# NVIDIA/audio-flamingo

Measured on AMD Instinct MI355X. Metric: audio-sec/s + decoder tokens/s, AF3-7B bf16 train, higher is better.
Workload: dtype bf16; 1 GPU; AF3 (AF-Whisper 32L + Qwen2.5-7B 28L, MLP projector) bf16 train step fwd+bwd+AdamW, 30 s clips, S=1024; micro_batch_per_gpu=8, global_batch=8, seq_len=1024, parallelism=dp1, activation_checkpointing=False

## Files before the change

### audio-flamingo_amd/csrc/attention_lds.hip

```cpp
#include "common.h"
#include "../../include/afk.h"

#ifdef AFK_PROBES
#define AFK_DBG(p) ((p).dbg)
#else
#define AFK_DBG(p) 0
#endif

namespace {

struct AttnArgs2 {
    const bf16* Q; int64_t q_bs, q_hs, q_rs;
    const bf16* K; int64_t k_bs, k_hs, k_rs;
    const bf16* V; int64_t v_bs, v_hs, v_rs;
    bf16* O; int64_t o_bs, o_hs, o_rs;
    const bf16* dO; int64_t do_bs, do_hs, do_rs;
    bf16* dQ; int64_t dq_bs, dq_hs, dq_rs;
    bf16* dK; int64_t dk_bs, dk_hs, dk_rs;
    bf16* dV; int64_t dv_bs, dv_hs, dv_rs;
    float* LSE;
    const float* delta;
    const int* kv_len;
    const int* kv_lo;
    int B, Hq, Hkv, S, Spad;
// ... 13 lines not shown
};

typedef __attribute__((address_space(3))) void lds_void;
typedef const __attribute__((address_space(1))) void gbl_void;
typedef __attribute__((address_space(3))) bf16x4 lds_bf16x4;

constexpr float NEG_INF = -INFINITY;
#define MFMA(a, b, c) __builtin_amdgcn_mfma_f32_32x32x16_bf16(a, b, c, 0, 0, 0)
#define ROW_OF(r, hi) (((r) & 3) + 8 * ((r) >> 2) + 4 * (hi))

__device__ __forceinline__ f32x16 zero16() {
    f32x16 z;
#pragma unroll
    for (int i = 0; i < 16; ++i) z[i] = 0.f;
    return z;
}

__device__ __forceinline__ float other_half(float x) {
    const unsigned u = __float_as_uint(x);
    const auto r = __builtin_amdgcn_permlane32_swap(u, u, false, false);
    return (threadIdx.x & 32) ? __uint_as_float(r[0]) : __uint_as_float(r[1]);
}
constexpr float LOG2E = 1.4426950408889634f, LN2 = 0.6931471805599453f;

template <bool WIDE>
__device__ __forceinline__ void store_block32(bf16* rowp, const f32x16& acc, float mul, int hi) {
    if constexpr (WIDE) {
#pragma unroll
        for (int t = 0; t < 2; ++t) {
            bf16x8 o;
#pragma unroll
            for (int e = 0; e < 4; ++e) {
                const auto r = __builtin_amdgcn_permlane32_swap(__float_as_uint(acc[8 * t + e]), __float_as_uint(acc[8 * t + 4 + e]), false, false);
                o[e] = (bf16)(__uint_as_float(r[0]) * mul);
                o[4 + e] = (bf16)(__uint_as_float(r[1]) * mul);
            }
            *(bf16x8*)(rowp + 16 * t + 8 * hi) = o;
        }
    } else {
#pragma unroll
        for (int qd = 0; qd < 4; ++qd) {
            bf16x4 o;
#pragma unroll
            for (int e = 0; e < 4; ++e) o[e] = (bf16)(acc[4 * qd + e] * mul);
            *(bf16x4*)(rowp + 8 * qd + 4 * hi) = o;
        }
// ... 140 lines not shown

#define AFK_ATTN_BARRIER()                                    \
    do {                                                      \
        asm volatile("s_waitcnt vmcnt(0)" ::: "memory");      \
        __builtin_amdgcn_sched_barrier(0);                    \
        __builtin_amdgcn_s_barrier();                         \
        __builtin_amdgcn_sched_barrier(0);                    \
    } while (0)
#define AFK_ATTN_BARRIER_P(p_)                                \
    do {                                                      \
        if (AFK_DBG(p_) & 16) {    \
            asm volatile("s_waitcnt vmcnt(0)" ::: "memory");  \
            __builtin_amdgcn_sched_barrier(0);                \
        } else if (AFK_DBG(p_) & 2) {                         \
            __builtin_amdgcn_sched_barrier(0);                \
            __builtin_amdgcn_s_barrier();                     \
            __builtin_amdgcn_sched_barrier(0);                \
        } else {                                              \
            AFK_ATTN_BARRIER();                               \
        }                                                     \
    } while (0)
constexpr float RESCALE_THR = 8.f;

template <int D, bool LM, int SCH>
__global__ __launch_bounds__(256, 2) void attn_fwd_lds_kernel(AttnArgs2 p) {
    using T = Tile<D>;
    constexpr int KS = T::KS, DT = T::DT;
    extern __shared__ __attribute__((aligned(16))) char smem[];
    const int lane = threadIdx.x & 63;
    const int wave = __builtin_amdgcn_readfirstlane(threadIdx.x >> 6);
    const int l31 = lane & 31, hi = lane >> 5;
    const typename T::Offs offs = T::make_offs(lane);
    const QBlock blk = attn_qblock(p);
    const int b = blk.b, h = blk.h, hk = h / (p.Hq / p.Hkv);
    const int qb0 = blk.z * 128;
    const int q0 = qb0 + wave * 32;
    const int q = q0 + l31;
    const int qc = min(q, p.S - 1);
    const int kv_len = p.kv_len ? min(p.kv_len[b], p.S) : p.S;
    const int kv_lo = p.kv_lo ? min(max(p.kv_lo[b], 0), kv_len) : 0;

    const bf16* Qp = p.Q + b * p.q_bs + h * p.q_hs + (int64_t)qc * p.q_rs + hi * 8;
    bf16x8 qf[KS];
#pragma unroll
    for (int ks = 0; ks < KS; ++ks) qf[ks] = *(const bf16x8*)(Qp + ks * 16);

    const bf16* Kbase = p.K + b * p.k_bs + hk * p.k_hs;
// ... 125 lines not shown
        float mx = fmaxf(st[0][0], st[1][0]);
#pragma unroll
        for (int r = 1; r < 16; ++r) mx = fmaxf(fmaxf(mx, st[0][r]), st[1][r]);
        mx = fmaxf(mx, other_half(mx)) * c2;
        if (__builtin_expect(__builtin_amdgcn_ballot_w64(mx > m + RESCALE_THR) != 0, 0)) {
            asm volatile("" ::);
            const float m_new = fmaxf(m, mx);
            const float alpha = __builtin_amdgcn_exp2f(m - ((m_new == NEG_INF) ? 0.f : m_new));
            if (LM) lacc[0] *= alpha;
            else l *= alpha;
#pragma unroll
            for (int dt = 0; dt < DT; ++dt)
#pragma unroll
                for (int r = 0; r < 16; ++r) oacc[dt][r] *= alpha;
            m = m_new;
        }
        const float nm = (m == NEG_INF) ? 0.f : -m;
        const f32x2 c2v = {c2, c2}, nmv = {nm, nm};
        f32x2 rs2 = {0.f, 0.f};
#pragma unroll
        for (int kt2 = 0; kt2 < 2; ++kt2)
#pragma unroll
            for (int r = 0; r < 16; r += 2) {
                const f32x2 s2 = {st[kt2][r], st[kt2][r + 1]};
                const f32x2 t2 = __builtin_elementwise_fma(s2, c2v, nmv);
                const f32x2 p2 = {__builtin_amdgcn_exp2f(t2[0]), __builtin_amdgcn_exp2f(t2[1])};
                if (!LM) rs2 += p2;
                pb[2 * kt2 + (r >> 3)][r & 7] = (bf16)p2[0];
                pb[2 * kt2 + (r >> 3)][(r & 7) + 1] = (bf16)p2[1];
            }
        if (!LM) l += rs2[0] + rs2[1];
        }
        if (LM) {
#pragma unroll
            for (int s4 = 0; s4 < 4; ++s4) lacc = MFMA(ones, pb[s4], lacc);
        }
        afk_frag_ring<DT>(issue, [&](auto g_, bf16x8(&f)[4]) {
            constexpr int dt = decltype(g_)::value;
#pragma unroll
            for (int s4 = 0; s4 < 4; ++s4) oacc[dt] = MFMA(f[s4], pb[s4], oacc[dt]);
        }, fa, fb);
    };

    const int j0 = kv_lo >> 6, j_int0 = (kv_lo + 63) >> 6;
    if (ntiles > j0) stage(j0);
    AFK_ATTN_BARRIER();
#pragma unroll
    for (int ks = 0; ks < KS; ++ks) asm volatile("" : "+v"(qf[ks]));
    int j = j0;
    constexpr std::false_type NO_DMA{};
// ... 242 lines not shown
            else l += other_half(l);
            const float inv = (l > 0.f) ? 1.f / l : 0.f;
            bf16* Op = p.O + bcur * p.o_bs + hcur * p.o_hs + (int64_t)qcur * p.o_rs;
            if (p.wide) {
#pragma unroll
                for (int dt = 0; dt < DT; ++dt) store_block32<true>(Op + dt * 32, oacc[dt], inv, hi);
            } else {
#pragma unroll
                for (int dt = 0; dt < DT; ++dt) store_block32<false>(Op + dt * 32, oacc[dt], inv, hi);
            }
            if (hi == 0 && p.LSE) p.LSE[((int64_t)bcur * p.Hq + hcur) * p.Spad + qcur] = (l > 0.f) ? -(m + __log2f(l)) / c2 : INFINITY;
        }
        if (!has_next) break;
    }
    if (threadIdx.x == 0 && !p.paired) {
        const int gone = __hip_atomic_fetch_add(queue + 1, 1, __ATOMIC_RELAXED, __HIP_MEMORY_SCOPE_AGENT);
        if (gone == (int)gridDim.x - 1) {
            __hip_atomic_store(queue, 0, __ATOMIC_RELAXED, __HIP_MEMORY_SCOPE_AGENT);
            __hip_atomic_store(queue + 1, 0, __ATOMIC_RELAXED, __HIP_MEMORY_SCOPE_AGENT);
        }
    }
}

template <int D, int SCH>
__global__ __launch_bounds__(256, 2) void attn_bwd_dq_lds_kernel(AttnArgs2 p) {
    using T = Tile<D>;
    constexpr int KS = T::KS, DT = T::DT;
    extern __shared__ __attribute__((aligned(16))) char smem[];
    const int lane = threadIdx.x & 63;
    const int wave = __builtin_amdgcn_readfirstlane(threadIdx.x >> 6);
    const int l31 = lane & 31, hi = lane >> 5;
    const typename T::Offs offs = T::make_offs(lane);
    const QBlock blk = attn_qblock(p);
    const int b = blk.b, h = blk.h, hk = h / (p.Hq / p.Hkv);
    const int qb0 = blk.z * 128;
    const int q0 = qb0 + wave * 32;
    const int q = q0 + l31;
    const int qc = min(q, p.S - 1);
    const int kv_len = p.kv_len ? min(p.kv_len[b], p.S) : p.S;
    const int kv_lo = p.kv_lo ? min(max(p.kv_lo[b], 0), kv_len) : 0;

    const bf16* Qp = p.Q + b * p.q_bs + h * p.q_hs + (int64_t)qc * p.q_rs + hi * 8;
    const bf16* dOp = p.dO + b * p.do_bs + h * p.do_hs + (int64_t)qc * p.do_rs + hi * 8;
    bf16x8 qf[KS], dof[KS];
#pragma unroll
    for (int ks = 0; ks < KS; ++ks) {
        qf[ks] = *(const bf16x8*)(Qp + ks * 16);
// ... 68 lines not shown
        constexpr bool isv = (i & 1) != 0;
        const uint32_t dst = lds0 + (jn & 1) * 2 * T::BYTES + wave * 1024 + (isv ? T::BYTES : 0) + 4 * u0 * 1024;
        if constexpr (isv) afk_dma16_saddr(Vbase + ((int64_t)jn * 64 + u0 * 4 * T::RPU) * p.v_rs, voff[0], dst);
        else afk_dma16_saddr(Kbase + ((int64_t)jn * 64 + u0 * 4 * T::RPU) * p.k_rs, koff[0], dst);
    };
    auto tile = [&](int j, auto masked_, auto par_, auto dma_) {
        constexpr bool MASKED = decltype(masked_)::value;
        constexpr bool DMA = decltype(dma_)::value;
        constexpr int POFF = par_static_off<decltype(par_)>(2 * T::BYTES);
        const uint32_t boff = par_dyn_off(par_, 2 * T::BYTES);
        const char* kimg = smem + POFF + boff;
        const char* vimg = kimg + T::BYTES;
        bf16x8 fa[4], fb[4];
        auto issue = [&](auto g_, bf16x8(&dst)[4]) {
            constexpr int dt = decltype(g_)::value;
            const uint32_t a0 = ktr[dt][0] + boff, a1 = ktr[dt][1] + boff;
            afk_static_for<4>([&](auto s_) { constexpr int s4 = decltype(s_)::value; dst[s4] = afk_lds_tr_frag<POFF + s4 * 16 * T::RS>(a0, a1); });
        };
        const f32x2 c2v = {c2, c2}, nl = {nlse, nlse}, nd = {ndlt, ndlt};
        bf16x8 dsb[4];
        auto ds_half = [&](int kt2, const f32x16& sh, const f32x16& dh) {
#pragma unroll
            for (int r = 0; r < 16; r += 2) {
                const f32x2 s2 = {sh[r], sh[r + 1]};
                const f32x2 t2 = __builtin_elementwise_fma(s2, c2v, nl);
                const f32x2 p2 = {__builtin_amdgcn_exp2f(t2[0]), __builtin_amdgcn_exp2f(t2[1])};
                const f32x2 d2 = {dh[r], dh[r + 1]};
                f32x2 ds2 = p2 * (d2 + nd);
                if (MASKED) {
                    const int key = j * 64 + kt2 * 32 + ROW_OF(r, hi);
                    if ((key >= kv_len) || (key < kv_lo) || (p.causal && key > q)) ds2[0] = 0.f;
                    if ((key + 1 >= kv_len) || (key + 1 < kv_lo) || (p.causal && key + 1 > q)) ds2[1] = 0.f;
                }
                dsb[2 * kt2 + (r >> 3)][r & 7] = (bf16)ds2[0];
                dsb[2 * kt2 + (r >> 3)][(r & 7) + 1] = (bf16)ds2[1];
            }
        };
        if constexpr (SCH == 0) {
            f32x16 st[2] = {zero16(), zero16()}, dp[2] = {zero16(), zero16()};
#pragma unroll
            for (int ks = 0; ks < KS; ++ks) {
                st[0] = MFMA(T::row_frag(kimg, offs, 0, ks), qf[ks], st[0]);
                st[1] = MFMA(T::row_frag(kimg, offs, 1, ks), qf[ks], st[1]);
                dp[0] = MFMA(T::row_frag(vimg, offs, 0, ks), dof[ks], dp[0]);
                dp[1] = MFMA(T::row_frag(vimg, offs, 1, ks), dof[ks], dp[1]);
            }
            issue(std::integral_constant<int, 0>{}, fa);
            ds_half(0, st[0], dp[0]);
            ds_half(1, st[1], dp[1]);
        } else {
            constexpr int NGK = KS / 2, NT = 2 * NGK, PPG = (2 * NP + NT - 1) / NT;
// ... 83 lines not shown
    if (q < p.S) {
        bf16* dQp = p.dQ + b * p.dq_bs + h * p.dq_hs + (int64_t)q * p.dq_rs;
        float mul = p.scale;
        if (p.rope_cos) {
            if (p.rope_cos_lanes && !p.rope_pos) {
                const int64_t rb = (int64_t)(q0 >> 5) * 32 * D;
                rope_bwd_rows<DT, true>(dqacc, mul, p.rope_cos_lanes + rb, p.rope_sin_lanes + rb, hi, l31);
            } else {
                const int64_t pr = p.rope_pos ? p.rope_pos[(int64_t)b * p.S + q] : q;
                rope_bwd_rows<DT>(dqacc, mul, p.rope_cos + pr * D, p.rope_sin + pr * D, hi);
            }
            mul = 1.f;
        }
        if (p.wide) {
#pragma unroll
            for (int dt = 0; dt < DT; ++dt) store_block32<true>(dQp + dt * 32, dqacc[dt], mul, hi);
        } else {
#pragma unroll
            for (int dt = 0; dt < DT; ++dt) store_block32<false>(dQp + dt * 32, dqacc[dt], mul, hi);
        }
    }
}

template <int D>
__global__ __launch_bounds__(256, (D <= 64 ? 2 : 1)) void attn_bwd_dkdv_lds_kernel(AttnArgs2 p) {
    using T = Tile<D>;
    constexpr int KS = T::KS, DT = T::DT;
    extern __shared__ __attribute__((aligned(16))) char smem[];
    uint64_t rt_entry = 0, rt1 = 0;
    if (AFK_DBG(p) & 4) asm volatile("s_memrealtime %0\n s_waitcnt lgkmcnt(0)" : "=s"(rt_entry)::"memory");
    const int lane = threadIdx.x & 63;
    const int wave = __builtin_amdgcn_readfirstlane(threadIdx.x >> 6);
    const int l31 = lane & 31, hi = lane >> 5;
    const typename T::Offs offs = T::make_offs(lane);
    const int b = blockIdx.y, group = p.Hq / p.Hkv;
    const int hy = blockIdx.x;
    const int P = p.split_heads;
    const int hk = P ? hy / P : hy;
    const int g_begin = P ? ((hy % P) * group) / P : 0;
    const int g_count = P ? (((hy % P) + 1) * group) / P - g_begin : group;
    const int kb0 = blockIdx.z * 128;
    const int key0 = kb0 + wave * 32;
    const int key = key0 + l31;
    const int keyc = min(key, p.S - 1);
    const int kv_len = p.kv_len ? min(p.kv_len[b], p.S) : p.S;
    const int kv_lo = p.kv_lo ? min(max(p.kv_lo[b], 0), kv_len) : 0;
    const bool wave_live = key0 < p.S;
// ... 50 lines not shown
            const uint32_t dst = lds0 + slot * BUF + wave * 1024;
#pragma unroll
            for (int u0 = 0; u0 < NP; ++u0) {
                afk_dma16_saddr(q0, qoff[u0], dst + 4 * u0 * 1024);
                afk_dma16_saddr(d0, dooff[u0], dst + T::BYTES + 4 * u0 * 1024);
            }
        } else {
            T::stage(buf, qb, p.q_rs, qt * 64, p.S - 1, wave, lane);
            T::stage(buf + T::BYTES, dob, p.do_rs, qt * 64, p.S - 1, wave, lane);
        }
        if (wave == 0)
            __builtin_amdgcn_global_load_lds((gbl_void*)(stat_lane + (int64_t)h * p.Spad + qt * 64), (lds_void*)(buf + STATS), 16, 0, 0);
    };

    uint64_t c_start = 0, ts0 = 0, ts1 = 0, ts2 = 0, tsm = 0, sum_body = 0, sum_ph1 = 0, sum_bar = 0, rt0 = 0;
    const bool probe = (AFK_DBG(p) & 4) != 0;
    uint32_t qrow[KS];
#pragma unroll
    for (int ks = 0; ks < KS; ++ks) qrow[ks] = lds0 + offs.row[ks];
    constexpr int NG = KS;
    constexpr int RD = (D == 128) ? 3 : 2;
    constexpr int PCH = 8 / NG;
    constexpr int SCH = 4 / DT;
    auto body = [&](int t, int qt, bool masked) {
        const uint32_t boff = (t & 1) * BUF;
        const float* stats = (const float*)(smem + boff + STATS) + 4 * hi;
        f32x16 st[2], dp[2];
#pragma unroll
        for (int qt2 = 0; qt2 < 2; ++qt2)
#pragma unroll
            for (int qd = 0; qd < 4; ++qd) {
                const f32x4 a = *(const f32x4*)(stats + qt2 * 32 + 8 * qd);
                const f32x4 d = *(const f32x4*)(stats + 64 + qt2 * 32 + 8 * qd);
#pragma unroll
                for (int e = 0; e < 4; ++e) {
                    st[qt2][4 * qd + e] = a[e];
                    dp[qt2][4 * qd + e] = d[e];
                }
            }
        bf16x8 r0[4], r1[4], r2[4];
        auto rbuf = [&](auto i_) -> bf16x8(&)[4] {
            constexpr int i = decltype(i_)::value;
            if constexpr (i == 0) return r0;
            else if constexpr (i == 1) return r1;
            else return r2;
        };
        auto issue_rows = [&](auto g_) {
            constexpr int G = decltype(g_)::value;
            constexpr int IMG = (G >= NG / 2) ? T::BYTES : 0, ks0 = (2 * G) % KS;
            bf16x8(&dst)[4] = rbuf(std::integral_constant<int, G % RD>{});
            const uint32_t a0 = qrow[ks0] + boff, a1 = qrow[ks0 + 1] + boff;
            dst[0] = afk_lds_b128<IMG>(a0);
            dst[1] = afk_lds_b128<IMG + 32 * T::RS>(a0);
            dst[2] = afk_lds_b128<IMG>(a1);
            dst[3] = afk_lds_b128<IMG + 32 * T::RS>(a1);
        };
        bf16x8 fa[4], fb[4];
        auto issue = [&](auto g_, bf16x8(&dst)[4]) {
            constexpr int g = decltype(g_)::value, dt = g % DT;
            constexpr int IMG = (g < DT) ? T::BYTES : 0;
            const uint32_t a0 = qtr[dt][0] + boff, a1 = qtr[dt][1] + boff;
            afk_static_for<4>([&](auto s_) { constexpr int s4 = decltype(s_)::value; dst[s4] = afk_lds_tr_frag<IMG + s4 * 16 * T::RS>(a0, a1); });
        };
        const f32x2 c2v = {c2, c2};
        bf16x8 pb[4], dsb[4];
        float pr[4][8];
        const int q_lo = key_dead ? p.S : (p.causal ? key : 0);
        auto p_chunk = [&](auto c_) {
            constexpr int c = decltype(c_)::value, qt2 = c >> 1, rb = 8 * (c & 1);
#pragma unroll
            for (int e = 0; e < 8; e += 2) {
                const f32x2 s2 = {st[qt2][rb + e], st[qt2][rb + e + 1]};
                const f32x2 t2 = s2 * c2v;
                pr[c][e] = __builtin_amdgcn_exp2f(t2[0]);
                pr[c][e + 1] = __builtin_amdgcn_exp2f(t2[1]);
            }
            if (masked) {
#pragma unroll
                for (int e = 0; e < 8; ++e) {
                    const int qq = qt * 64 + qt2 * 32 + 8 * ((rb + e) >> 2) + 4 * hi + ((rb + e) & 3);
                    if (qq < q_lo || qq >= p.S) pr[c][e] = 0.f;
                }
            }
#pragma unroll
            for (int e = 0; e < 8; ++e) pb[c][e] = (bf16)pr[c][e];
        };
        auto ds_chunk = [&](auto c_) {
            constexpr int c = decltype(c_)::value, qt2 = c >> 1, rb = 8 * (c & 1);
#pragma unroll
            for (int e = 0; e < 8; e += 2) {
                const f32x2 p2 = {pr[c][e], pr[c][e + 1]};
                const f32x2 d2 = {dp[qt2][rb + e], dp[qt2][rb + e + 1]};
                const f32x2 ds2 = p2 * d2;
                dsb[c][e] = (bf16)ds2[0];
                dsb[c][e + 1] = (bf16)ds2[1];
            }
        };

        afk_static_for<RD - 1>([&](auto g_) { issue_rows(g_); });
        afk_static_for<NG>([&](auto g_) {
            constexpr int G = decltype(g_)::value;
            bf16x8(&cur)[4] = rbuf(std::integral_constant<int, G % RD>{});
            if constexpr (G + RD - 1 < NG) {
                issue_rows(std::integral_constant<int, G + RD - 1>{});
                afk_lgkmcnt<4 * (RD - 1)>();
            } else if constexpr (G + 1 < NG) {
                afk_lgkmcnt<4 * (NG - 1 - G)>();
            } else {
                afk_lgkmcnt<8>();
            }
            afk_lds_tie(cur[0], cur[1], cur[2], cur[3]);
            constexpr int ks0 = (2 * G) % KS;
            if constexpr (G < NG / 2) {
                st[0] = MFMA(cur[0], kf[ks0], st[0]);
                st[1] = MFMA(cur[1], kf[ks0], st[1]);
                st[0] = MFMA(cur[2], kf[ks0 + 1], st[0]);
// ... 8 lines not shown
            if constexpr (G >= NG / 2)
                afk_static_for<PCH>([&](auto i_) { p_chunk(std::integral_constant<int, (G - NG / 2) * PCH + decltype(i_)::value>{}); });
        });
        if (AFK_DBG(p) & 8) {
            asm volatile("s_waitcnt lgkmcnt(0)\n s_memtime %0\n s_waitcnt lgkmcnt(0)" : "=s"(tsm)::"memory");
            sum_ph1 += tsm - ts0;
        }
        afk_frag_ring<2 * DT>(issue, [&](auto g_, bf16x8(&f)[4]) {
            constexpr int g = decltype(g_)::value, dt = g % DT;
#pragma unroll
            for (int s4 = 0; s4 < 4; ++s4) {
                if (g < DT) dvacc[dt] = MFMA(f[s4], pb[s4], dvacc[dt]);
                else dkacc[dt] = MFMA(f[s4], dsb[s4], dkacc[dt]);
            }
            if constexpr (g < DT) afk_static_for<SCH>([&](auto i_) { ds_chunk(std::integral_constant<int, g * SCH + decltype(i_)::value>{}); });
        }, fa, fb);
    };

    const int h0 = hk * group + g_begin;
    if (ntiles > 0) stage(0, h0, qt_begin);
    AFK_ATTN_BARRIER();
    if (probe) asm volatile("s_memtime %0\n s_memrealtime %1\n s_waitcnt lgkmcnt(0)" : "=s"(c_start), "=s"(rt0)::"memory");
    int t = 0;
    for (int gi = 0; gi < (block_dead ? 0 : g_count); ++gi) {
        const int h = h0 + gi;
        for (int qt = qt_begin; qt < qt_end; ++qt, ++t) {
            {
                const bool wrap = qt + 1 == qt_end;
                const bool last = wrap && gi + 1 == g_count;
                const int nh = (wrap && !last) ? h + 1 : h, nqt = last ? qt : (wrap ? qt_begin : qt + 1);
                if (!(AFK_DBG(p) & 1) || t < 1) stage((t + 1) & 1, nh, nqt);
            }
            const bool interior = qt >= qt_int0 && qt < qt_int1;
            if (probe) asm volatile("s_memtime %0\n s_waitcnt lgkmcnt(0)" : "=s"(ts0)::"memory");
            if (!(AFK_DBG(p) & 2) && (interior || (wave_live && !(p.causal && qt * 64 + 63 < key0)))) body(t, qt, !interior);
            if (probe) asm volatile("s_memtime %0\n s_waitcnt lgkmcnt(0)" : "=s"(ts1)::"memory");
            AFK_ATTN_BARRIER();
            if (probe) {
                asm volatile("s_memtime %0\n s_waitcnt lgkmcnt(0)" : "=s"(ts2)::"memory");
                sum_body += ts1 - ts0;
                sum_bar += ts2 - ts1;
            }
        }
    }
    uint64_t c_end = 0;
    if (probe) {
        asm volatile("s_memtime %0\n s_memrealtime %1\n s_waitcnt lgkmcnt(0)" : "=s"(c_end), "=s"(rt1)::"memory");
        if (lane == 0) {
            float* o = (float*)p.dQ + ((((int64_t)blockIdx.z * gridDim.y + blockIdx.y) * gridDim.x + blockIdx.x) * 4 + wave) * 8;
            o[0] = (float)(c_end - c_start); o[1] = (float)sum_body; o[2] = (float)sum_bar; o[3] = (float)ntiles;
            o[4] = (float)(rt1 - rt0); o[5] = (float)sum_ph1; o[6] = (float)blockIdx.z;
        }
    }
    if (key < p.S) {
        bf16* dKp = p.dK + b * p.dk_bs + hy * p.dk_hs + (int64_t)key * p.dk_rs;
        bf16* dVp = p.dV + b * p.dv_bs + hy * p.dv_hs + (int64_t)key * p.dv_rs;
        float kmul = p.scale;
        if (p.rope_cos && !p.split_heads) {
// ... 151 lines not shown
        const int64_t t = i >> 8;
        const int j = (int)(t % PH), h2 = (int)((t / PH) & 1);
        const int64_t rb = t / PH / 2;
        const int64_t r = rb * 32 + l31;
        out[i] = r < rows ? tab[r * D + h2 * (D / 2) + 8 * j + 4 * hi + e] : (bf16)0.f;
    }
}

bool attn_wide_stores() {
    static const bool on = [] { const char* e = getenv("AFK_ATTN_WIDE"); return !(e && e[0] == '0'); }();
    return on;
}

int g_persist_paired = 0;
int g_xcd_map = -1;
int attn_xcd_map() {
    if (g_xcd_map < 0) {
        const char* e = getenv("AFK_ATTN_XCD");
        g_xcd_map = e ? (atoi(e) != 0) : 1;
    }
    return g_xcd_map;
}
int g_dkdv_parts = 0;
int g_attn_sched = -1;
int attn_sched() {
    if (g_attn_sched < 0) {
        const char* e = getenv("AFK_ATTN_SCHED");
        g_attn_sched = e ? (atoi(e) != 0) : 1;
    }
    return g_attn_sched;
}

template <typename K>
int set_lds(K kern, int bytes) {
    return hipFuncSetAttribute((const void*)kern, hipFuncAttributeMaxDynamicSharedMemorySize, bytes) == hipSuccess ? 0 : 1;
}

}

extern "C" int afk_attn2_fwd(const void* Q, int64_t q_bs, int64_t q_hs, int64_t q_rs, const void* K, int64_t k_bs, int64_t k_hs,
                             int64_t k_rs, const void* V, int64_t v_bs, int64_t v_hs, int64_t v_rs, void* O, int64_t o_bs,
                             int64_t o_hs, int64_t o_rs, float* LSE, const int* kv_len, const int* kv_lo, int B, int Hq, int Hkv, int S, int Spad,
                             int D, float scale, int causal, void* stream) {
    AFK_REQUIRE(Q && K && V && O && LSE, "afk_attn2_fwd: null pointer");
    AFK_REQUIRE(B > 0 && Hq > 0 && Hkv > 0 && Hq % Hkv == 0 && S > 0 && Spad >= S && Spad % 64 == 0, "afk_attn2_fwd: bad shape");
    AFK_REQUIRE(D == 64 || D == 128, "afk_attn2_fwd: head_dim %d unsupported by the LDS kernels (64/128)", D);
// ... 2 lines not shown
    AttnArgs2 p = {};
    p.Q = (const bf16*)Q; p.q_bs = q_bs; p.q_hs = q_hs; p.q_rs = q_rs;
    p.K = (const bf16*)K; p.k_bs = k_bs; p.k_hs = k_hs; p.k_rs = k_rs;
    p.V = (const bf16*)V; p.v_bs = v_bs; p.v_hs = v_hs; p.v_rs = v_rs;
    p.O = (bf16*)O; p.o_bs = o_bs; p.o_hs = o_hs; p.o_rs = o_rs;
    AFK_REQUIRE(!kv_lo || causal, "afk_attn2_fwd: kv_lo (left padding) is defined for causal attention only");
    p.LSE = LSE; p.kv_len = kv_len; p.kv_lo = kv_lo;
    p.B = B; p.Hq = Hq; p.Hkv = Hkv; p.S = S; p.Spad = Spad; p.scale = scale; p.causal = causal;
    p.wide = attn_wide_stores() && (uintptr_t)O % 16 == 0 && o_bs % 8 == 0 && o_hs % 8 == 0 && o_rs % 8 == 0;
    p.nz = (int)afk_cdiv(S, 128);
    p.xcd_map = attn_xcd_map();
#ifdef AFK_PROBES
    {
        static const char* dbg = getenv("AFK_ATTN_DBG");
        if (dbg) p.dbg = atoi(dbg);
    }
#endif
    dim3 grid((unsigned)Hq, (unsigned)B, (unsigned)p.nz);
    if (p.xcd_map) grid = dim3((unsigned)(Hq * B * p.nz));
    hipStream_t st = (hipStream_t)stream;
    afk_count(D == 128 ? AFK_CNT_ATTN2_FWD_D128 : AFK_CNT_ATTN2_FWD_D64);
    static const int lsum_env = [] { const char* e = getenv("AFK_ATTN_LSUM"); return e ? (e[0] == '1' ? 1 : 0) : -1; }();
    const bool lm = lsum_env < 0 ? D == 128 : lsum_env == 1;
#define AFK_FWD(DD, LM_, SCH_)                                                                      \
    do {                                                                                            \
        constexpr int L = 4 * Tile<DD>::BYTES;                                                      \
        static int once = set_lds(attn_fwd_lds_kernel<DD, LM_, SCH_>, L);                           \
        (void)once;                                                                                 \
        hipLaunchKernelGGL((attn_fwd_lds_kernel<DD, LM_, SCH_>), grid, dim3(256), L, st, p);        \
    } while (0)
    const int sch = attn_sched();
    if (D == 128) {
        if (sch) { if (lm) AFK_FWD(128, true, 1); else AFK_FWD(128, false, 1); }
        else { if (lm) AFK_FWD(128, true, 0); else AFK_FWD(128, false, 0); }
    } else {
        if (sch) { if (lm) AFK_FWD(64, true, 1); else AFK_FWD(64, false, 1); }
        else { if (lm) AFK_FWD(64, true, 0); else AFK_FWD(64, false, 0); }
    }
#undef AFK_FWD
    AFK_LAUNCH_CHECK("afk_attn2_fwd");
    return AFK_OK;
}

extern "C" int afk_attn_set_sched(int sched) {
    AFK_REQUIRE(sched == 0 || sched == 1, "afk_attn_set_sched: 0 or 1");
    g_attn_sched = sched;
    return AFK_OK;
}

extern "C" int afk_attn_set_persist_paired(int on) {
    AFK_REQUIRE(on == 0 || on == 1, "afk_attn_set_persist_paired: 0 or 1");
    g_persist_paired = on;
    return AFK_OK;
}

extern "C" int afk_attn_set_xcd_map(int on) {
    AFK_REQUIRE(on == 0 || on == 1, "afk_attn_set_xcd_map: 0 or 1");
    g_xcd_map = on;
    return AFK_OK;
}

extern "C" int afk_attn_set_dkdv_parts(int parts) {
    AFK_REQUIRE(parts >= 0 && parts <= 64, "afk_attn_set_dkdv_parts: 0 (environment / default) or the number of dK/dV partials per kv head");
    g_dkdv_parts = parts;
    return AFK_OK;
}

extern "C" int afk_attn2_fwd_persistent(const void* Q, int64_t q_bs, int64_t q_hs, int64_t q_rs, const void* K, int64_t k_bs, int64_t k_hs,
                                        int64_t k_rs, const void* V, int64_t v_bs, int64_t v_hs, int64_t v_rs, void* O, int64_t o_bs,
                                        int64_t o_hs, int64_t o_rs, float* LSE, const int* kv_len, const int* kv_lo, int B, int Hq, int Hkv, int S, int Spad,
                                        int D, float scale, int causal, int* queue, void* stream) {
    if (kv_len || kv_lo || S % 128 != 0 || !queue)
        return afk_attn2_fwd(Q, q_bs, q_hs, q_rs, K, k_bs, k_hs, k_rs, V, v_bs, v_hs, v_rs, O, o_bs, o_hs, o_rs, LSE, kv_len, kv_lo, B, Hq, Hkv, S, Spad, D, scale, causal, stream);
    AFK_REQUIRE(Q && K && V && O && LSE, "afk_attn2_fwd_persistent: null pointer");
    AFK_REQUIRE(B > 0 && Hq > 0 && Hkv > 0 && Hq % Hkv == 0 && Spad >= S && Spad % 64 == 0 && (D == 64 || D == 128), "afk_attn2_fwd_persistent: bad shape");
    AFK_REQUIRE(q_rs % 8 == 0 && k_rs % 8 == 0 && v_rs % 8 == 0 && q_hs % 8 == 0 && k_hs % 8 == 0 && v_hs % 8 == 0 && o_rs % 4 == 0,
                "afk_attn2_fwd_persistent: strides must keep 16-byte alignment");
    AttnArgs2 p = {};
    p.Q = (const bf16*)Q; p.q_bs = q_bs; p.q_hs = q_hs; p.q_rs = q_rs;
    p.K = (const bf16*)K; p.k_bs = k_bs; p.k_hs = k_hs; p.k_rs = k_rs;
    p.V = (const bf16*)V; p.v_bs = v_bs; p.v_hs = v_hs; p.v_rs = v_rs;
// ... 93 lines not shown
    if (split) {
        const int64_t per_part = (int64_t)B * Hkv * afk_cdiv(S, 128);
        int want = g_dkdv_parts > 0 ? g_dkdv_parts : parts_env;
        if (want <= 0) want = (int)std::min<int64_t>(group, std::max<int64_t>(1, afk_cdiv(512, per_part)));
        P = std::max(1, std::min(group, want));
    }
    const bool direct = split && P == 1;
    if (split && !direct) {
        pk.split_heads = P;
        pk.dK = (bf16*)gqa_scratch;
        pk.dV = (bf16*)gqa_scratch + (int64_t)B * S * Hq * D;
        pk.dk_bs = pk.dv_bs = (int64_t)S * Hkv * P * D;
        pk.dk_hs = pk.dv_hs = D;
        pk.dk_rs = pk.dv_rs = (int64_t)Hkv * P * D;
    }
    afk_count(D == 128 ? AFK_CNT_ATTN2_BWD_D128 : AFK_CNT_ATTN2_BWD_D64);
    if (split && !direct) afk_count(AFK_CNT_GQA_REDUCE);
    dim3 gkv((unsigned)(split && !direct ? Hkv * P : Hkv), (unsigned)B, (unsigned)afk_cdiv(S, 128));
    p.nz = pk.nz = (int)afk_cdiv(S, 128);
    p.xcd_map = attn_xcd_map();
    dim3 gq((unsigned)Hq, (unsigned)B, (unsigned)p.nz);
    if (p.xcd_map) gq = dim3((unsigned)(Hq * B * p.nz));
    const int sch = attn_sched();
    auto launch_dq = [&](auto d_) {
        constexpr int DD = decltype(d_)::value;
        constexpr int L = 4 * Tile<DD>::BYTES;
        if (sch) hipLaunchKernelGGL((attn_bwd_dq_lds_kernel<DD, 1>), gq, dim3(256), L, st, p);
        else hipLaunchKernelGGL((attn_bwd_dq_lds_kernel<DD, 0>), gq, dim3(256), L, st, p);
    };
    if (D == 128) {
        constexpr int L = 4 * Tile<128>::BYTES, LKV = L + 2048;
        static int once = set_lds(attn_bwd_dkdv_lds_kernel<128>, LKV) + set_lds(attn_bwd_dq_lds_kernel<128, 0>, L) + set_lds(attn_bwd_dq_lds_kernel<128, 1>, L);
        (void)once;
        if (O) launch_dq(std::integral_constant<int, 128>{});
        hipLaunchKernelGGL(attn_bwd_dkdv_lds_kernel<128>, gkv, dim3(256), LKV, st, pk);
        if (!O && !(AFK_DBG(p) & 4)) launch_dq(std::integral_constant<int, 128>{});
    } else {
        constexpr int L = 4 * Tile<64>::BYTES, LKV = L + 2048;
        static int once = set_lds(attn_bwd_dkdv_lds_kernel<64>, LKV) + set_lds(attn_bwd_dq_lds_kernel<64, 0>, L) + set_lds(attn_bwd_dq_lds_kernel<64, 1>, L);
        (void)once;
        if (O) launch_dq(std::integral_constant<int, 64>{});
        hipLaunchKernelGGL(attn_bwd_dkdv_lds_kernel<64>, gkv, dim3(256), LKV, st, pk);
        if (!O && !(AFK_DBG(p) & 4)) launch_dq(std::integral_constant<int, 64>{});
    }
    if (split && !direct && !(AFK_DBG(p) & 4)) {
        AFK_REQUIRE(dk_hs == D && dv_hs == D && dk_bs == (int64_t)S * dk_rs && dv_bs == (int64_t)S * dv_rs && dk_rs == dv_rs,
                    "afk_attn2_bwd: GQA split path expects dK/dV inside one [B*S, ld] buffer with contiguous heads");
        const int64_t rows = (int64_t)B * S;
        int g = (int)afk_cdiv(rows * (Hkv * D / 8), 256);
        if (g > 4096) g = 4096;
        if (rope_cos) {
            const int64_t items = rows * (Hkv * D / 16) + rows * (Hkv * D / 8);
            int g2 = (int)std::min<int64_t>(afk_cdiv(items, 256), 4096);
            hipLaunchKernelGGL(gqa_reduce_rope_kernel, dim3(g2), dim3(256), 0, st, pk.dK, pk.dV, (bf16*)dK, (bf16*)dV, rows, Hkv, P, D, dk_rs, dv_rs,
                               (const bf16*)rope_cos, (const bf16*)rope_sin, rope_pos, S);
        } else {
            hipLaunchKernelGGL(gqa_reduce_kernel, dim3(g), dim3(256), 0, st, pk.dK, (bf16*)dK, rows, Hkv, P, D, dk_rs);
            hipLaunchKernelGGL(gqa_reduce_kernel, dim3(g), dim3(256), 0, st, pk.dV, (bf16*)dV, rows, Hkv, P, D, dv_rs);
        }
    }
    AFK_LAUNCH_CHECK("afk_attn2_bwd");
    return AFK_OK;
}

extern "C" int afk_attn2_bwd(const void* Q, int64_t q_bs, int64_t q_hs, int64_t q_rs, const void* K, int64_t k_bs, int64_t k_hs,
                             int64_t k_rs, const void* V, int64_t v_bs, int64_t v_hs, int64_t v_rs, const void* dO, int64_t do_bs,
                             int64_t do_hs, int64_t do_rs, const float* LSE, const float* delta, void* dQ, int64_t dq_bs,
// ... 40 lines not shown
```

### include/afk.h

```cpp
#ifndef AFK_H
#define AFK_H
#include <stdint.h>
#ifdef __cplusplus
extern "C" {
#endif

int afk_version(void);
const char* afk_last_error(void);
const char* afk_build_id(void);
int afk_has_probes(void);

#define AFK_CNT_GEMM_NT128 0
#define AFK_CNT_GEMM_NT256 1
#define AFK_CNT_GEMM_NN256 2
#define AFK_CNT_GEMM_TN256 3
#define AFK_CNT_GEMM_SPLITK 4
#define AFK_CNT_GEMV 5
#define AFK_CNT_ATTN2_FWD_D64 6
#define AFK_CNT_ATTN2_FWD_D128 7
#define AFK_CNT_ATTN2_BWD_D64 8
#define AFK_CNT_ATTN2_BWD_D128 9
#define AFK_CNT_GQA_REDUCE 10
#define AFK_CNT_XATTN_FWD 11
#define AFK_CNT_XATTN_BWD 12
// ... 100 lines not shown
                 int64_t dv_rs, const int* kv_len, int B, int Hq, int Hkv, int S, int Spad, int D, float scale,
                 int causal, void* stream);

int afk_xattn_fwd(const void* Q, int64_t q_bs, int64_t q_hs, int64_t q_rs, const void* K, int64_t k_bs, int64_t k_hs,
                  int64_t k_rs, const void* Vt, void* O, int64_t o_bs, int64_t o_hs, int64_t o_rs, float* LSE,
                  const int* kv_len, const int* krange, int B, int Hq, int Hkv, int Sq, int Sk, int Sqpad, int Skpad,
                  int D, float scale, void* stream);
int afk_xattn_bwd(const void* Q, int64_t q_bs, int64_t q_hs, int64_t q_rs, const void* K, int64_t k_bs, int64_t k_hs,
                  int64_t k_rs, const void* V, int64_t v_bs, int64_t v_hs, int64_t v_rs, const void* dO,
                  int64_t do_bs, int64_t do_hs, int64_t do_rs, const void* Qt, const void* Kt, const void* dOt,
                  const float* LSE, const float* delta, void* dQ, int64_t dq_bs, int64_t dq_hs, int64_t dq_rs,
                  void* dK, int64_t dk_bs, int64_t dk_hs, int64_t dk_rs, void* dV, int64_t dv_bs, int64_t dv_hs,
                  int64_t dv_rs, const int* kv_len, const int* krange, int B, int Hq, int Hkv, int Sq, int Sk,
                  int Sqpad, int Skpad, int D, float scale, void* stream);

int afk_attn2_fwd(const void* Q, int64_t q_bs, int64_t q_hs, int64_t q_rs, const void* K, int64_t k_bs, int64_t k_hs,
                  int64_t k_rs, const void* V, int64_t v_bs, int64_t v_hs, int64_t v_rs, void* O, int64_t o_bs,
                  int64_t o_hs, int64_t o_rs, float* LSE, const int* kv_len, const int* kv_lo, int B, int Hq, int Hkv, int S, int Spad,
                  int D, float scale, int causal, void* stream);
int afk_attn_set_sched(int sched);
int afk_attn_set_xcd_map(int on);
int afk_attn_set_persist_paired(int on);
int afk_attn_set_dkdv_parts(int parts);
int afk_attn2_fwd_persistent(const void* Q, int64_t q_bs, int64_t q_hs, int64_t q_rs, const void* K, int64_t k_bs, int64_t k_hs,
                             int64_t k_rs, const void* V, int64_t v_bs, int64_t v_hs, int64_t v_rs, void* O, int64_t o_bs,
                             int64_t o_hs, int64_t o_rs, float* LSE, const int* kv_len, const int* kv_lo, int B, int Hq, int Hkv, int S, int Spad,
                             int D, float scale, int causal, int* queue, void* stream);
int afk_attn2_delta(const void* O, int64_t o_bs, int64_t o_hs, int64_t o_rs, const void* dO, int64_t do_bs, int64_t do_hs,
                    int64_t do_rs, float* delta, int B, int H, int S, int Spad, int D, void* stream);
int afk_attn2_bwd(const void* Q, int64_t q_bs, int64_t q_hs, int64_t q_rs, const void* K, int64_t k_bs, int64_t k_hs,
                  int64_t k_rs, const void* V, int64_t v_bs, int64_t v_hs, int64_t v_rs, const void* dO, int64_t do_bs,
                  int64_t do_hs, int64_t do_rs, const float* LSE, const float* delta, void* dQ, int64_t dq_bs,
                  int64_t dq_hs, int64_t dq_rs, void* dK, int64_t dk_bs, int64_t dk_hs, int64_t dk_rs, void* dV,
                  int64_t dv_bs, int64_t dv_hs, int64_t dv_rs, const int* kv_len, const int* kv_lo, int B, int Hq, int Hkv, int S,
                  int Spad, int D, float scale, int causal, void* gqa_scratch, void* stream);
int afk_attn2_bwd_fused(const void* Q, int64_t q_bs, int64_t q_hs, int64_t q_rs, const void* K, int64_t k_bs, int64_t k_hs,
                        int64_t k_rs, const void* V, int64_t v_bs, int64_t v_hs, int64_t v_rs, const void* O, int64_t o_bs, int64_t o_hs,
                        int64_t o_rs, const void* dO, int64_t do_bs, int64_t do_hs, int64_t do_rs, const float* LSE, float* delta_ws,
                        void* dQ, int64_t dq_bs, int64_t dq_hs, int64_t dq_rs, void* dK, int64_t dk_bs, int64_t dk_hs, int64_t dk_rs,
                        void* dV, int64_t dv_bs, int64_t dv_hs, int64_t dv_rs, const int* kv_len, const int* kv_lo, int B, int Hq,
                        int Hkv, int S, int Spad, int D, float scale, int causal, void* gqa_scratch, void* stream);
int afk_attn2_bwd_fused_rope(const void* Q, int64_t q_bs, int64_t q_hs, int64_t q_rs, const void* K, int64_t k_bs, int64_t k_hs,
                             int64_t k_rs, const void* V, int64_t v_bs, int64_t v_hs, int64_t v_rs, const void* O, int64_t o_bs, int64_t o_hs,
                             int64_t o_rs, const void* dO, int64_t do_bs, int64_t do_hs, int64_t do_rs, const float* LSE, float* delta_ws,
                             void* dQ, int64_t dq_bs, int64_t dq_hs, int64_t dq_rs, void* dK, int64_t dk_bs, int64_t dk_hs, int64_t dk_rs,
                             void* dV, int64_t dv_bs, int64_t dv_hs, int64_t dv_rs, const int* kv_len, const int* kv_lo, int B, int Hq,
// ... 167 lines not shown
```

Baseline: 636.4 audio-s/s.

## Add static-slot unmasked dK/dV loop and scalar VALU softmax forms

Adds a FORM=1 path in the dK/dV backward kernel that splits the q-tile loop into dead, masked and fully unmasked ranges. Unmasked tiles are processed in pairs with compile-time LDS buffer slots and direct DMA staging via pointer increments, which removes dynamic buffer offsets and mask checks from the hot loop. It also adds a VF template option that computes the exp/FMA softmax math as scalar ops instead of packed f32x2, using asm barriers to stop the compiler from re-packing them. Both are on by default (FORM=1, scalar VALU only for dK/dV with D=64), which adds template instantiations and more complex control flow.

After: 637.9 audio-s/s (median of 6 runs). Within noise of the previous version (+0.2%).

```diff
diff --git a/audio-flamingo_amd/csrc/attention_lds.hip b/audio-flamingo_amd/csrc/attention_lds.hip
--- a/audio-flamingo_amd/csrc/attention_lds.hip
+++ b/audio-flamingo_amd/csrc/attention_lds.hip
@@ -59,6 +59,10 @@
     return (threadIdx.x & 32) ? __uint_as_float(r[0]) : __uint_as_float(r[1]);
 }
 constexpr float LOG2E = 1.4426950408889634f, LN2 = 0.6931471805599453f;
+__device__ __forceinline__ float afk_unpacked(float x) {
+    asm("" : "+v"(x));
+    return x;
+}
 
 template <bool WIDE>
 __device__ __forceinline__ void store_block32(bf16* rowp, const f32x16& acc, float mul, int hi) {
@@ -245,7 +249,7 @@
     } while (0)
 constexpr float RESCALE_THR = 8.f;
 
-template <int D, bool LM, int SCH>
+template <int D, bool LM, int SCH, int VF>
 __global__ __launch_bounds__(256, 2) void attn_fwd_lds_kernel(AttnArgs2 p) {
     using T = Tile<D>;
     constexpr int KS = T::KS, DT = T::DT;
@@ -417,10 +421,21 @@
         for (int kt2 = 0; kt2 < 2; ++kt2)
 #pragma unroll
             for (int r = 0; r < 16; r += 2) {
-                const f32x2 s2 = {st[kt2][r], st[kt2][r + 1]};
-                const f32x2 t2 = __builtin_elementwise_fma(s2, c2v, nmv);
-                const f32x2 p2 = {__builtin_amdgcn_exp2f(t2[0]), __builtin_amdgcn_exp2f(t2[1])};
-                if (!LM) rs2 += p2;
+                f32x2 p2;
+                if constexpr (VF == 0) {
+                    const f32x2 s2 = {st[kt2][r], st[kt2][r + 1]};
+                    const f32x2 t2 = __builtin_elementwise_fma(s2, c2v, nmv);
+                    p2[0] = __builtin_amdgcn_exp2f(t2[0]);
+                    p2[1] = __builtin_amdgcn_exp2f(t2[1]);
+                    if (!LM) rs2 += p2;
+                } else {
+                    p2[0] = __builtin_amdgcn_exp2f(afk_unpacked(__builtin_fmaf(st[kt2][r], c2, nm)));
+                    p2[1] = __builtin_amdgcn_exp2f(afk_unpacked(__builtin_fmaf(st[kt2][r + 1], c2, nm)));
+                    if (!LM) {
+                        rs2[0] = afk_unpacked(rs2[0] + p2[0]);
+                        rs2[1] = afk_unpacked(rs2[1] + p2[1]);
+                    }
+                }
                 pb[2 * kt2 + (r >> 3)][r & 7] = (bf16)p2[0];
                 pb[2 * kt2 + (r >> 3)][(r & 7) + 1] = (bf16)p2[1];
             }
@@ -709,7 +724,7 @@
     }
 }
 
-template <int D, int SCH>
+template <int D, int SCH, int VF>
 __global__ __launch_bounds__(256, 2) void attn_bwd_dq_lds_kernel(AttnArgs2 p) {
     using T = Tile<D>;
     constexpr int KS = T::KS, DT = T::DT;
@@ -824,11 +839,20 @@
         auto ds_half = [&](int kt2, const f32x16& sh, const f32x16& dh) {
 #pragma unroll
             for (int r = 0; r < 16; r += 2) {
-                const f32x2 s2 = {sh[r], sh[r + 1]};
-                const f32x2 t2 = __builtin_elementwise_fma(s2, c2v, nl);
-                const f32x2 p2 = {__builtin_amdgcn_exp2f(t2[0]), __builtin_amdgcn_exp2f(t2[1])};
-                const f32x2 d2 = {dh[r], dh[r + 1]};
-                f32x2 ds2 = p2 * (d2 + nd);
+                f32x2 ds2;
+                if constexpr (VF == 0) {
+                    const f32x2 s2 = {sh[r], sh[r + 1]};
+                    const f32x2 t2 = __builtin_elementwise_fma(s2, c2v, nl);
+                    const f32x2 p2 = {__builtin_amdgcn_exp2f(t2[0]), __builtin_amdgcn_exp2f(t2[1])};
+                    const f32x2 d2 = {dh[r], dh[r + 1]};
+                    ds2 = p2 * (d2 + nd);
+                } else {
+#pragma unroll
+                    for (int e = 0; e < 2; ++e) {
+                        const float pe = __builtin_amdgcn_exp2f(afk_unpacked(__builtin_fmaf(sh[r + e], c2, nlse)));
+                        ds2[e] = afk_unpacked(pe * afk_unpacked(dh[r + e] + ndlt));
+                    }
+                }
                 if (MASKED) {
                     const int key = j * 64 + kt2 * 32 + ROW_OF(r, hi);
                     if ((key >= kv_len) || (key < kv_lo) || (p.causal && key > q)) ds2[0] = 0.f;
@@ -958,7 +982,7 @@
     }
 }
 
-template <int D>
+template <int D, int FORM, int VF>
 __global__ __launch_bounds__(256, (D <= 64 ? 2 : 1)) void attn_bwd_dkdv_lds_kernel(AttnArgs2 p) {
     using T = Tile<D>;
     constexpr int KS = T::KS, DT = T::DT;
@@ -1055,9 +1079,11 @@
     constexpr int RD = (D == 128) ? 3 : 2;
     constexpr int PCH = 8 / NG;
     constexpr int SCH = 4 / DT;
-    auto body = [&](int t, int qt, bool masked) {
-        const uint32_t boff = (t & 1) * BUF;
-        const float* stats = (const float*)(smem + boff + STATS) + 4 * hi;
+    auto body = [&](auto par_, int qt, auto masked_) {
+        using PAR = decltype(par_);
+        constexpr int SOFF = par_static_off<PAR>(BUF);
+        const uint32_t boff = par_dyn_off(par_, BUF);
+        const float* stats = (const float*)(smem + SOFF + boff + STATS) + 4 * hi;
         f32x16 st[2], dp[2];
 #pragma unroll
         for (int qt2 = 0; qt2 < 2; ++qt2)
@@ -1083,17 +1109,17 @@
             constexpr int IMG = (G >= NG / 2) ? T::BYTES : 0, ks0 = (2 * G) % KS;
             bf16x8(&dst)[4] = rbuf(std::integral_constant<int, G % RD>{});
             const uint32_t a0 = qrow[ks0] + boff, a1 = qrow[ks0 + 1] + boff;
-            dst[0] = afk_lds_b128<IMG>(a0);
-            dst[1] = afk_lds_b128<IMG + 32 * T::RS>(a0);
-            dst[2] = afk_lds_b128<IMG>(a1);
-            dst[3] = afk_lds_b128<IMG + 32 * T::RS>(a1);
+            dst[0] = afk_lds_b128<SOFF + IMG>(a0);
+            dst[1] = afk_lds_b128<SOFF + IMG + 32 * T::RS>(a0);
+            dst[2] = afk_lds_b128<SOFF + IMG>(a1);
+            dst[3] = afk_lds_b128<SOFF + IMG + 32 * T::RS>(a1);
         };
         bf16x8 fa[4], fb[4];
         auto issue = [&](auto g_, bf16x8(&dst)[4]) {
             constexpr int g = decltype(g_)::value, dt = g % DT;
             constexpr int IMG = (g < DT) ? T::BYTES : 0;
             const uint32_t a0 = qtr[dt][0] + boff, a1 = qtr[dt][1] + boff;
-            afk_static_for<4>([&](auto s_) { constexpr int s4 = decltype(s_)::value; dst[s4] = afk_lds_tr_frag<IMG + s4 * 16 * T::RS>(a0, a1); });
+            afk_static_for<4>([&](auto s_) { constexpr int s4 = decltype(s_)::value; dst[s4] = afk_lds_tr_frag<SOFF + IMG + s4 * 16 * T::RS>(a0, a1); });
         };
         const f32x2 c2v = {c2, c2};
         bf16x8 pb[4], dsb[4];
@@ -1103,17 +1129,27 @@
             constexpr int c = decltype(c_)::value, qt2 = c >> 1, rb = 8 * (c & 1);
 #pragma unroll
             for (int e = 0; e < 8; e += 2) {
-                const f32x2 s2 = {st[qt2][rb + e], st[qt2][rb + e + 1]};
-                const f32x2 t2 = s2 * c2v;
-                pr[c][e] = __builtin_amdgcn_exp2f(t2[0]);
-                pr[c][e + 1] = __builtin_amdgcn_exp2f(t2[1]);
-            }
+                if constexpr (VF == 0) {
+                    const f32x2 s2 = {st[qt2][rb + e], st[qt2][rb + e + 1]};
+                    const f32x2 t2 = s2 * c2v;
+                    pr[c][e] = __builtin_amdgcn_exp2f(t2[0]);
+                    pr[c][e + 1] = __builtin_amdgcn_exp2f(t2[1]);
+                } else {
+                    pr[c][e] = __builtin_amdgcn_exp2f(afk_unpacked(st[qt2][rb + e] * c2));
+                    pr[c][e + 1] = __builtin_amdgcn_exp2f(afk_unpacked(st[qt2][rb + e + 1] * c2));
+                }
+            }
+            bool masked;
+            if constexpr (std::is_same<decltype(masked_), bool>::value) masked = masked_;
+            else masked = decltype(masked_)::value;
             if (masked) {
+                if constexpr (!std::is_same<decltype(masked_), bool>::value) __builtin_amdgcn_sched_barrier(0);
 #pragma unroll
                 for (int e = 0; e < 8; ++e) {
                     const int qq = qt * 64 + qt2 * 32 + 8 * ((rb + e) >> 2) + 4 * hi + ((rb + e) & 3);
                     if (qq < q_lo || qq >= p.S) pr[c][e] = 0.f;
                 }
+                if constexpr (!std::is_same<decltype(masked_), bool>::value) __builtin_amdgcn_sched_barrier(0);
             }
 #pragma unroll
             for (int e = 0; e < 8; ++e) pb[c][e] = (bf16)pr[c][e];
@@ -1122,9 +1158,15 @@
             constexpr int c = decltype(c_)::value, qt2 = c >> 1, rb = 8 * (c & 1);
 #pragma unroll
             for (int e = 0; e < 8; e += 2) {
-                const f32x2 p2 = {pr[c][e], pr[c][e + 1]};
-                const f32x2 d2 = {dp[qt2][rb + e], dp[qt2][rb + e + 1]};
-                const f32x2 ds2 = p2 * d2;
+                f32x2 ds2;
+                if constexpr (VF == 0) {
+                    const f32x2 p2 = {pr[c][e], pr[c][e + 1]};
+                    const f32x2 d2 = {dp[qt2][rb + e], dp[qt2][rb + e + 1]};
+                    ds2 = p2 * d2;
+                } else {
+                    ds2[0] = afk_unpacked(pr[c][e] * dp[qt2][rb + e]);
+                    ds2[1] = afk_unpacked(pr[c][e + 1] * dp[qt2][rb + e + 1]);
+                }
                 dsb[c][e] = (bf16)ds2[0];
                 dsb[c][e + 1] = (bf16)ds2[1];
             }
@@ -1179,6 +1221,82 @@
     AFK_ATTN_BARRIER();
     if (probe) asm volatile("s_memtime %0\n s_memrealtime %1\n s_waitcnt lgkmcnt(0)" : "=s"(c_start), "=s"(rt0)::"memory");
     int t = 0;
+    if constexpr (FORM == 1) {
+        const uint32_t dma_dst = lds0 + wave * 1024;
+        const int64_t q_step = 64 * p.q_rs, do_step = 64 * p.do_rs;
+        auto stage_full = [&](auto slot_, const bf16* q0, const bf16* d0, const float* st0) {
+            constexpr int SLOT = decltype(slot_)::value;
+#pragma unroll
+            for (int u0 = 0; u0 < NP; ++u0) {
+                afk_dma16_saddr(q0, qoff[u0], dma_dst + SLOT * BUF + 4 * u0 * 1024);
+                afk_dma16_saddr(d0, dooff[u0], dma_dst + SLOT * BUF + T::BYTES + 4 * u0 * 1024);
+            }
+            if (wave == 0) __builtin_amdgcn_global_load_lds((gbl_void*)st0, (lds_void*)(smem + SLOT * BUF + STATS), 16, 0, 0);
+        };
+        constexpr std::integral_constant<int, 0> SLOT0{};
+        constexpr std::integral_constant<int, 1> SLOT1{};
+        auto slow_tile = [&](int h, bool last_head, int qt, auto run_) {
+            const bool wrap = qt + 1 == qt_end;
+            const bool last = wrap && last_head;
+            const int nh = (wrap && !last) ? h + 1 : h, nqt = last ? qt : (wrap ? qt_begin : qt + 1);
+            if (!(AFK_DBG(p) & 1) || t < 1) stage((t + 1) & 1, nh, nqt);
+            if (probe) asm volatile("s_memtime %0\n s_waitcnt lgkmcnt(0)" : "=s"(ts0)::"memory");
+            if constexpr (decltype(run_)::value) body(DynPar{t & 1}, qt, std::true_type{});
+            if (probe) asm volatile("s_memtime %0\n s_waitcnt lgkmcnt(0)" : "=s"(ts1)::"memory");
+            AFK_ATTN_BARRIER();
+            if (probe) {
+                asm volatile("s_memtime %0\n s_waitcnt lgkmcnt(0)" : "=s"(ts2)::"memory");
+                sum_body += ts1 - ts0;
+                sum_bar += ts2 - ts1;
+            }
+        };
+        const int n_dead = ((AFK_DBG(p) & 2) || !wave_live) ? qt_end : (p.causal ? key0 >> 6 : 0);
+        for (int gi = 0; gi < (block_dead ? 0 : g_count); ++gi) {
+            const int h = h0 + gi;
+            const bool last_head = gi + 1 == g_count;
+            const int f0 = qt_int0 + ((t + qt_int0 - qt_begin) & 1);
+            const int f1 = f0 + (max(qt_int1 - f0, 0) & ~1);
+            int qt = qt_begin;
+            for (; qt < min(n_dead, qt_end); ++qt, ++t) slow_tile(h, last_head, qt, std::false_type{});
+            for (const int lead_end = f1 > f0 ? f0 : qt_end; qt < lead_end; ++qt, ++t) slow_tile(h, last_head, qt, std::true_type{});
+            {
+                if (f1 > f0 && qt == f0) {
+                    const bool wrap = f1 == qt_end;
+                    const int nh = (wrap && !last_head) ? h + 1 : h, nqt = (wrap && last_head) ? f1 - 1 : (wrap ? qt_begin : f1);
+                    const bf16* qp = p.Q + b * p.q_bs + h * p.q_hs + (int64_t)(f0 + 1) * q_step;
+                    const bf16* dop = p.dO + b * p.do_bs + h * p.do_hs + (int64_t)(f0 + 1) * do_step;
+                    const float* stp = stat_lane + (int64_t)h * p.Spad + (f0 + 1) * 64;
+                    for (; qt < f1; qt += 2) {
+                        stage_full(SLOT1, qp, dop, stp);
+                        if (probe) asm volatile("s_memtime %0\n s_waitcnt lgkmcnt(0)" : "=s"(ts0)::"memory");
+                        body(StaticPar<0>{}, qt, std::false_type{});
+                        if (probe) asm volatile("s_memtime %0\n s_waitcnt lgkmcnt(0)" : "=s"(ts1)::"memory");
+                        AFK_ATTN_BARRIER();
+                        if (probe) {
+                            asm volatile("s_memtime %0\n s_waitcnt lgkmcnt(0)" : "=s"(ts2)::"memory");
+                            sum_body += ts1 - ts0;
+                            sum_bar += ts2 - ts1;
+                        }
+                        qp += q_step; dop += do_step; stp += 64;
+                        if (__builtin_expect(qt + 2 < f1, 1)) stage_full(SLOT0, qp, dop, stp);
+                        else stage(0, nh, nqt);
+                        if (probe) asm volatile("s_memtime %0\n s_waitcnt lgkmcnt(0)" : "=s"(ts0)::"memory");
+                        body(StaticPar<1>{}, qt + 1, std::false_type{});
+                        if (probe) asm volatile("s_memtime %0\n s_waitcnt lgkmcnt(0)" : "=s"(ts1)::"memory");
+                        AFK_ATTN_BARRIER();
+                        if (probe) {
+                            asm volatile("s_memtime %0\n s_waitcnt lgkmcnt(0)" : "=s"(ts2)::"memory");
+                            sum_body += ts1 - ts0;
+                            sum_bar += ts2 - ts1;
+                        }
+                        qp += q_step; dop += do_step; stp += 64;
+                    }
+                    t += f1 - f0;
+                }
+            }
+            for (; qt < qt_end; ++qt, ++t) slow_tile(h, last_head, qt, std::true_type{});
+        }
+    } else
     for (int gi = 0; gi < (block_dead ? 0 : g_count); ++gi) {
         const int h = h0 + gi;
         for (int qt = qt_begin; qt < qt_end; ++qt, ++t) {
@@ -1190,7 +1308,7 @@
             }
             const bool interior = qt >= qt_int0 && qt < qt_int1;
             if (probe) asm volatile("s_memtime %0\n s_waitcnt lgkmcnt(0)" : "=s"(ts0)::"memory");
-            if (!(AFK_DBG(p) & 2) && (interior || (wave_live && !(p.causal && qt * 64 + 63 < key0)))) body(t, qt, !interior);
+            if (!(AFK_DBG(p) & 2) && (interior || (wave_live && !(p.causal && qt * 64 + 63 < key0)))) body(DynPar{t & 1}, qt, !interior);
             if (probe) asm volatile("s_memtime %0\n s_waitcnt lgkmcnt(0)" : "=s"(ts1)::"memory");
             AFK_ATTN_BARRIER();
             if (probe) {
@@ -1388,6 +1506,26 @@
     return g_xcd_map;
 }
 int g_dkdv_parts = 0;
+int g_dkdv_form = -1;
+int attn_dkdv_form() {
+    if (g_dkdv_form < 0) {
+        const char* e = getenv("AFK_ATTN_DKDV_FORM");
+        g_dkdv_form = e ? (atoi(e) != 0) : 1;
+    }
+    return g_dkdv_form;
+}
+enum { VALU_FWD = 2, VALU_DQ = 3, VALU_DKDV = 4 };
+int g_valu_form = -2;
+int attn_valu_form(int kernel, int D) {
+    if (g_valu_form == -2) {
+        const char* e = getenv("AFK_ATTN_VALU_FORM");
+        const int v = e ? atoi(e) : -1;
+        g_valu_form = (v >= 0 && v <= 4) ? v : -1;
+    }
+    if (g_valu_form == 0 || g_valu_form == 1) return g_valu_form;
+    if (g_valu_form >= 2) return g_valu_form == kernel;
+    return kernel == VALU_DKDV && D == 64;
+}
 int g_attn_sched = -1;
 int attn_sched() {
     if (g_attn_sched < 0) {
@@ -1436,12 +1574,18 @@
     afk_count(D == 128 ? AFK_CNT_ATTN2_FWD_D128 : AFK_CNT_ATTN2_FWD_D64);
     static const int lsum_env = [] { const char* e = getenv("AFK_ATTN_LSUM"); return e ? (e[0] == '1' ? 1 : 0) : -1; }();
     const bool lm = lsum_env < 0 ? D == 128 : lsum_env == 1;
+#define AFK_FWD_VF(DD, LM_, SCH_, VF_)                                                              \
+    do {                                                                                            \
+        constexpr int L = 4 * Tile<DD>::BYTES;                                                      \
+        static int once = set_lds(attn_fwd_lds_kernel<DD, LM_, SCH_, VF_>, L);                      \
+        (void)once;                                                                                 \
+        hipLaunchKernelGGL((attn_fwd_lds_kernel<DD, LM_, SCH_, VF_>), grid, dim3(256), L, st, p);   \
+    } while (0)
+    const int vf = attn_valu_form(VALU_FWD, D);
 #define AFK_FWD(DD, LM_, SCH_)                                                                      \
     do {                                                                                            \
-        constexpr int L = 4 * Tile<DD>::BYTES;                                                      \
-        static int once = set_lds(attn_fwd_lds_kernel<DD, LM_, SCH_>, L);                           \
-        (void)once;                                                                                 \
-        hipLaunchKernelGGL((attn_fwd_lds_kernel<DD, LM_, SCH_>), grid, dim3(256), L, st, p);        \
+        if (vf) AFK_FWD_VF(DD, LM_, SCH_, 1);                                                       \
+        else AFK_FWD_VF(DD, LM_, SCH_, 0);                                                          \
     } while (0)
     const int sch = attn_sched();
     if (D == 128) {
@@ -1452,6 +1596,7 @@
         else { if (lm) AFK_FWD(64, true, 0); else AFK_FWD(64, false, 0); }
     }
 #undef AFK_FWD
+#undef AFK_FWD_VF
     AFK_LAUNCH_CHECK("afk_attn2_fwd");
     return AFK_OK;
 }
@@ -1471,6 +1616,18 @@
 extern "C" int afk_attn_set_xcd_map(int on) {
     AFK_REQUIRE(on == 0 || on == 1, "afk_attn_set_xcd_map: 0 or 1");
     g_xcd_map = on;
+    return AFK_OK;
+}
+
+extern "C" int afk_attn_set_dkdv_form(int form) {
+    AFK_REQUIRE(form == 0 || form == 1, "afk_attn_set_dkdv_form: 0 or 1");
+    g_dkdv_form = form;
+    return AFK_OK;
+}
+
+extern "C" int afk_attn_set_valu_form(int form) {
+    AFK_REQUIRE(form >= -1 && form <= 4, "afk_attn_set_valu_form: -1 (per-kernel default), 0 packed, 1 scalar, 2 / 3 / 4 scalar in forward / dQ / dK/dV only");
+    g_valu_form = form;
     return AFK_OK;
 }
 
@@ -1610,27 +1767,43 @@
     dim3 gq((unsigned)Hq, (unsigned)B, (unsigned)p.nz);
     if (p.xcd_map) gq = dim3((unsigned)(Hq * B * p.nz));
     const int sch = attn_sched();
+    const int form = attn_dkdv_form();
+    const int vf_dq = attn_valu_form(VALU_DQ, D), vf_kv = attn_valu_form(VALU_DKDV, D);
     auto launch_dq = [&](auto d_) {
         constexpr int DD = decltype(d_)::value;
         constexpr int L = 4 * Tile<DD>::BYTES;
-        if (sch) hipLaunchKernelGGL((attn_bwd_dq_lds_kernel<DD, 1>), gq, dim3(256), L, st, p);
-        else hipLaunchKernelGGL((attn_bwd_dq_lds_kernel<DD, 0>), gq, dim3(256), L, st, p);
+        auto go = [&](auto sch_, auto vf_) {
+            constexpr int SC = decltype(sch_)::value, VF = decltype(vf_)::value;
+            static int once = set_lds(attn_bwd_dq_lds_kernel<DD, SC, VF>, L);
+            (void)once;
+            hipLaunchKernelGGL((attn_bwd_dq_lds_kernel<DD, SC, VF>), gq, dim3(256), L, st, p);
+        };
+        constexpr std::integral_constant<int, 0> I0{};
+        constexpr std::integral_constant<int, 1> I1{};
+        if (sch) { if (vf_dq) go(I1, I1); else go(I1, I0); }
+        else { if (vf_dq) go(I0, I1); else go(I0, I0); }
     };
-    if (D == 128) {
-        constexpr int L = 4 * Tile<128>::BYTES, LKV = L + 2048;
-        static int once = set_lds(attn_bwd_dkdv_lds_kernel<128>, LKV) + set_lds(attn_bwd_dq_lds_kernel<128, 0>, L) + set_lds(attn_bwd_dq_lds_kernel<128, 1>, L);
-        (void)once;
-        if (O) launch_dq(std::integral_constant<int, 128>{});
-        hipLaunchKernelGGL(attn_bwd_dkdv_lds_kernel<128>, gkv, dim3(256), LKV, st, pk);
-        if (!O && !(AFK_DBG(p) & 4)) launch_dq(std::integral_constant<int, 128>{});
-    } else {
-        constexpr int L = 4 * Tile<64>::BYTES, LKV = L + 2048;
-        static int once = set_lds(attn_bwd_dkdv_lds_kernel<64>, LKV) + set_lds(attn_bwd_dq_lds_kernel<64, 0>, L) + set_lds(attn_bwd_dq_lds_kernel<64, 1>, L);
-        (void)once;
-        if (O) launch_dq(std::integral_constant<int, 64>{});
-        hipLaunchKernelGGL(attn_bwd_dkdv_lds_kernel<64>, gkv, dim3(256), LKV, st, pk);
-        if (!O && !(AFK_DBG(p) & 4)) launch_dq(std::integral_constant<int, 64>{});
-    }
+    auto launch_dkdv = [&](auto d_) {
+        constexpr int DD = decltype(d_)::value;
+        constexpr int LKV = 4 * Tile<DD>::BYTES + 2048;
+        auto go = [&](auto form_, auto vf_) {
+            constexpr int FM = decltype(form_)::value, VF = decltype(vf_)::value;
+            static int once = set_lds(attn_bwd_dkdv_lds_kernel<DD, FM, VF>, LKV);
+            (void)once;
+            hipLaunchKernelGGL((attn_bwd_dkdv_lds_kernel<DD, FM, VF>), gkv, dim3(256), LKV, st, pk);
+        };
+        constexpr std::integral_constant<int, 0> I0{};
+        constexpr std::integral_constant<int, 1> I1{};
+        if (form) { if (vf_kv) go(I1, I1); else go(I1, I0); }
+        else { if (vf_kv) go(I0, I1); else go(I0, I0); }
+    };
+    auto launch_all = [&](auto d_) {
+        if (O) launch_dq(d_);
+        launch_dkdv(d_);
+        if (!O && !(AFK_DBG(p) & 4)) launch_dq(d_);
+    };
+    if (D == 128) launch_all(std::integral_constant<int, 128>{});
+    else launch_all(std::integral_constant<int, 64>{});
     if (split && !direct && !(AFK_DBG(p) & 4)) {
         AFK_REQUIRE(dk_hs == D && dv_hs == D && dk_bs == (int64_t)S * dk_rs && dv_bs == (int64_t)S * dv_rs && dk_rs == dv_rs,
                     "afk_attn2_bwd: GQA split path expects dK/dV inside one [B*S, ld] buffer with contiguous heads");
diff --git a/include/afk.h b/include/afk.h
--- a/include/afk.h
+++ b/include/afk.h
@@ -146,6 +146,8 @@
 int afk_attn_set_xcd_map(int on);
 int afk_attn_set_persist_paired(int on);
 int afk_attn_set_dkdv_parts(int parts);
+int afk_attn_set_dkdv_form(int form);
+int afk_attn_set_valu_form(int form);
 int afk_attn2_fwd_persistent(const void* Q, int64_t q_bs, int64_t q_hs, int64_t q_rs, const void* K, int64_t k_bs, int64_t k_hs,
                              int64_t k_rs, const void* V, int64_t v_bs, int64_t v_hs, int64_t v_rs, void* O, int64_t o_bs,
                              int64_t o_hs, int64_t o_rs, float* LSE, const int* kv_len, const int* kv_lo, int B, int Hq, int Hkv, int S, int Spad,
```
